# linnil1/KIR_graph

Hardware: AMD Instinct MI355X
Metric: typed 150 bp PE reads/s (pileup+EM) per GPU; achieved HBM GB/s vs roofline (higher is better)
Workload: dtype f64

## Files before the change

kir_graph_amd/csrc/gk_rowclass.hip:

```cpp
#include "gk_rowclass.h"

namespace {

constexpr int kThreads = 256;
constexpr int kGroup = 16, kDeep = 4;
constexpr int kRound = kGroup * kDeep;
constexpr int kCap = 256;
constexpr uint64_t kEmptyKey = ~0ull;
constexpr int kExpandCols = 8;

__device__ inline uint64_t mix64(uint64_t x) {
  x ^= x >> 30; x *= 0xBF58476D1CE4E5B9ull;
  x ^= x >> 27; x *= 0x94D049BB133111EBull;
  return x ^ (x >> 31);
}

template <class F>
__device__ inline uint32_t walk_round(const uint32_t* __restrict__ ids, const uint8_t* __restrict__ vflag, uint32_t k0,
                                      uint32_t mid, uint32_t e, int lane, int shift, uint32_t kept_before, F&& f) {
  uint32_t v[kDeep];
  uint8_t fl[kDeep];
  const uint32_t last = e - 1u;
#pragma unroll
  for (int j = 0; j < kDeep; ++j) {
    const uint32_t k = k0 + (uint32_t)lane + kGroup * j;
    v[j] = ids[k < e ? k : last];
  }
#pragma unroll
  for (int j = 0; j < kDeep; ++j) fl[j] = vflag[v[j]];
  uint32_t run = kept_before;
#pragma unroll
  for (int j = 0; j < kDeep; ++j) {
    const uint32_t k = k0 + (uint32_t)lane + kGroup * j;
    const bool positive = k < mid;
    const bool keep = k < e && !(fl[j] & (positive ? 1 : 2));
    const uint32_t mine = (uint32_t)(__ballot(keep) >> shift) & 0xFFFFu;
    if (keep) f((v[j] << 1) | (positive ? 0u : 1u), run + (uint32_t)__builtin_popcount(mine & ((1u << lane) - 1u)));
    run += (uint32_t)__builtin_popcount(mine);
  }
  return run;
}

__global__ __launch_bounds__(kThreads) void rowclass_keys(const int32_t* __restrict__ rows, int64_t n_rows,
                                                          const uint32_t* __restrict__ off,
                                                          const uint32_t* __restrict__ ids,
                                                          const uint8_t* __restrict__ vflag, uint64_t hash_mask,
                                                          unsigned long long* slot_key, uint32_t* slot_rep,
                                                          uint32_t slot_mask, uint32_t* __restrict__ slot_of) {
  const int lane = threadIdx.x & (kGroup - 1);
  const int shift = (threadIdx.x & 63) & ~(kGroup - 1);
  const int64_t i = ((int64_t)blockIdx.x * kThreads + threadIdx.x) / kGroup;
  const bool active = i < n_rows;
  uint32_t b = 0, mid = 0, e = 0;
  if (active) {
    const int64_t row = rows[i];
    b = off[4 * row]; mid = off[4 * row + 2]; e = off[4 * row + 4];
  }
  uint64_t h = 0;
  uint32_t n = 0;
  for (uint32_t k0 = b; k0 < e; k0 += kRound)
    n = walk_round(ids, vflag, k0, mid, e, lane, shift, n,
                   [&](uint32_t token, uint32_t rank) { h += mix64(((uint64_t)rank << 32) | token); });
  uint32_t lo = (uint32_t)h, hi = (uint32_t)(h >> 32);
#pragma unroll
  for (int d = kGroup / 2; d > 0; d >>= 1) {
    const uint64_t o = ((uint64_t)(uint32_t)__shfl_xor((int)hi, d, 64) << 32) | (uint32_t)__shfl_xor((int)lo, d, 64);
    h += o;
    lo = (uint32_t)h; hi = (uint32_t)(h >> 32);
  }
  if (!active || lane != 0) return;
  const unsigned long long key = mix64(h ^ n) & hash_mask & ~(1ull << 63);
  uint32_t s = (uint32_t)(key ^ (key >> 32)) & slot_mask;
  for (;;) {
    unsigned long long prev = __hip_atomic_load(&slot_key[s], __ATOMIC_RELAXED, __HIP_MEMORY_SCOPE_AGENT);
    if (prev == kEmptyKey) prev = atomicCAS(&slot_key[s], (unsigned long long)kEmptyKey, key);
    if (prev == kEmptyKey || prev == key) break;
    s = (s + 1u) & slot_mask;
  }
  if (__hip_atomic_load(&slot_rep[s], __ATOMIC_RELAXED, __HIP_MEMORY_SCOPE_AGENT) > (uint32_t)i)
    atomicMin(&slot_rep[s], (uint32_t)i);
  slot_of[i] = s;
}

__global__ __launch_bounds__(kThreads) void rowclass_verify(const int32_t* __restrict__ rows, int64_t n_rows,
                                                            const uint32_t* __restrict__ off,
                                                            const uint32_t* __restrict__ ids,
                                                            const uint8_t* __restrict__ vflag,
                                                            const uint32_t* __restrict__ slot_rep,
                                                            const uint32_t* __restrict__ slot_of,
                                                            uint32_t* __restrict__ is_rep, uint32_t* __restrict__ rep_of) {
  __shared__ uint32_t kept[kThreads / kGroup][kCap];
  const int lane = threadIdx.x & (kGroup - 1);
  const int shift = (threadIdx.x & 63) & ~(kGroup - 1);
  const int g = threadIdx.x / kGroup;
  const int64_t i = ((int64_t)blockIdx.x * kThreads + threadIdx.x) / kGroup;
  const bool active = i < n_rows;
  const uint32_t rep = active ? slot_rep[slot_of[i]] : 0u;
  const bool compare = active && rep < (uint32_t)i;
  uint32_t b = 0, mid = 0, e = 0, rb = 0, rmid = 0, re = 0;
  if (compare) {
    const int64_t row = rows[i], rrow = rows[rep];
    b = off[4 * row]; mid = off[4 * row + 2]; e = off[4 * row + 4];
    rb = off[4 * rrow]; rmid = off[4 * rrow + 2]; re = off[4 * rrow + 4];
  }
  uint32_t* const mine = kept[g];
  uint32_t n = 0, rn = 0;
  for (uint32_t k0 = b; k0 < e; k0 += kRound)
    n = walk_round(ids, vflag, k0, mid, e, lane, shift, n, [&](uint32_t token, uint32_t rank) {
      if (rank < (uint32_t)kCap) mine[rank] = token;
    });
  __builtin_amdgcn_fence(__ATOMIC_RELEASE, "wavefront");
  __builtin_amdgcn_wave_barrier();
  __builtin_amdgcn_fence(__ATOMIC_ACQUIRE, "wavefront");
  bool differs = false;
  for (uint32_t k0 = rb; k0 < re; k0 += kRound)
    rn = walk_round(ids, vflag, k0, rmid, re, lane, shift, rn, [&](uint32_t token, uint32_t rank) {
      if (rank < (uint32_t)kCap && mine[rank] != token) differs = true;
    });
  const bool any = ((__ballot(differs) >> shift) & 0xFFFFull) != 0ull;
  const bool same = compare && n == rn && n <= (uint32_t)kCap && !any;
  if (active && lane == 0) {
    is_rep[i] = same ? 0u : 1u;
    rep_of[i] = same ? rep : (uint32_t)i;
  }
}

__global__ __launch_bounds__(kThreads) void rowclass_rank(const int32_t* __restrict__ rep_idx,
                                                          const uint32_t* __restrict__ n_classes, int64_t n_rows,
                                                          const int32_t* __restrict__ rows, uint32_t* __restrict__ rank_of,
                                                          int32_t* __restrict__ rep_rows) {
  const int64_t c = (int64_t)blockIdx.x * kThreads + threadIdx.x;
  if (c >= n_rows || c >= (int64_t)*n_classes) return;
  const int32_t r = rep_idx[c];
  rank_of[r] = (uint32_t)c;
  rep_rows[c] = rows[r];
}

__global__ __launch_bounds__(kThreads) void rowclass_classof(const uint32_t* __restrict__ rep_of,
                                                             const uint32_t* __restrict__ rank_of, int64_t n_rows,
                                                             uint32_t* __restrict__ class_of) {
  const int64_t i = (int64_t)blockIdx.x * kThreads + threadIdx.x;
  if (i < n_rows) class_of[i] = rank_of[rep_of[i]];
}

__global__ __launch_bounds__(kThreads) void rowclass_expand(const double* __restrict__ Lc, int64_t ldc,
                                                            const uint32_t* __restrict__ class_of, int64_t n_rows,
                                                            int n_cols, double* __restrict__ L,
                                                            uint8_t* __restrict__ miss8, int64_t ldm) {
  const int a0 = (int)blockIdx.y * kExpandCols;
  const int n_a = min(kExpandCols, n_cols - a0);
  const int64_t r0 = 4 * ((int64_t)blockIdx.x * kThreads + threadIdx.x);
  if (r0 >= ldm) return;
  if (r0 >= n_rows) {
    for (int a = 0; a < n_a; ++a) *reinterpret_cast<uint32_t*>(miss8 + (int64_t)(a0 + a) * ldm + r0) = 0u;
    return;
  }
  const int n_r = (int)(n_rows - r0 < 4 ? n_rows - r0 : 4);
  uint32_t c[4];
  if (n_r == 4) {
    const uint4 q = *reinterpret_cast<const uint4*>(class_of + r0);
    c[0] = q.x; c[1] = q.y; c[2] = q.z; c[3] = q.w;
  } else {
#pragma unroll
    for (int j = 0; j < 4; ++j) c[j] = class_of[j < n_r ? r0 + j : n_rows - 1];
  }
  double v[4][kExpandCols];
#pragma unroll
  for (int j = 0; j < 4; ++j) {
    const double2* const src = reinterpret_cast<const double2*>(Lc + (int64_t)c[j] * ldc + a0);
#pragma unroll
    for (int q = 0; q < kExpandCols / 2; ++q) {
      const double2 x = src[q];
      v[j][2 * q] = x.x; v[j][2 * q + 1] = x.y;
    }
  }
#pragma unroll
  for (int a = 0; a < kExpandCols; ++a) {
    if (a >= n_a) break;
    uint32_t packed = 0;
#pragma unroll
    for (int j = 0; j < 4; ++j) {
      const double t = __builtin_fma(v[j][a], -1.0 / 3.0, 0.25);
      const uint32_t m = t < 100.0 ? (uint32_t)(int)t : 255u;
      if (j < n_r) packed |= m << (8 * j);
    }
    double* const dst = L + (int64_t)(a0 + a) * n_rows + r0;
    if (n_r == 4) {
#pragma unroll
      for (int j = 0; j < 4; ++j) dst[j] = v[j][a];
    } else {
#pragma unroll
      for (int j = 0; j < 4; ++j)
        if (j < n_r) dst[j] = v[j][a];
    }
    *reinterpret_cast<uint32_t*>(miss8 + (int64_t)(a0 + a) * ldm + r0) = packed;
  }
}

inline unsigned nblk(int64_t n) { return (unsigned)((n + kThreads - 1) / kThreads); }

}

int64_t gk_rowclass_ld(int n_cols) { return ((int64_t)n_cols + kExpandCols - 1) / kExpandCols * kExpandCols; }

int gk_rowclass_enqueue(gk_ctx* ctx, gk_tab* tab, const int32_t* d_rows, int64_t n_rows, const uint8_t* d_vflag,
                        gk_rowclass* rc) {
  GK_REQUIRE(ctx && tab && rc && d_rows && d_vflag && n_rows > 0 && n_rows <= 0x7FFFFFFFll, "bad row-class arguments");
  hipStream_t st = ctx->stream;
  const long bits = gk_test_hook_value("rowclass_hashbits", 63);
  const uint64_t hash_mask = bits >= 63 ? ~0ull : bits <= 0 ? 0ull : (1ull << bits) - 1ull;
  uint64_t n_slots = 64;
  while (n_slots < 2 * (uint64_t)n_rows) n_slots <<= 1;
  GkBlocks temps(ctx);
  char* slots = nullptr;
  uint32_t *slot_of = nullptr, *is_rep = nullptr, *rep_of = nullptr, *rank_of = nullptr, *class_of = nullptr, *n_classes = nullptr;
  int32_t *rep_idx = nullptr, *rep_rows = nullptr;
  const size_t per_row = (size_t)n_rows * sizeof(uint32_t);
  if (temps.take(&slots, (size_t)n_slots * 12) != hipSuccess || temps.take(&slot_of, per_row) != hipSuccess ||
      temps.take(&is_rep, per_row) != hipSuccess || temps.take(&rep_of, per_row) != hipSuccess ||
      temps.take(&rank_of, per_row) != hipSuccess || temps.take(&rep_idx, per_row) != hipSuccess ||
      temps.take(&rep_rows, per_row) != hipSuccess || temps.take(&class_of, per_row) != hipSuccess) {
    gk_set_error("out of device memory for the row classes");
    return GK_ERR_HIP;
  }
  unsigned long long* const slot_key = reinterpret_cast<unsigned long long*>(slots);
  uint32_t* const slot_rep = reinterpret_cast<uint32_t*>(slots + (size_t)n_slots * 8);
  if (hipMemsetAsync(slots, 0xFF, (size_t)n_slots * 12, st) != hipSuccess) {
    gk_set_error("row classes: clearing the slots failed");
    return GK_ERR_HIP;
  }
  const unsigned groups = nblk(n_rows * kGroup);
  GK_PROF(ctx, "rowclass_keys", GK_KERNEL(rowclass_keys, dim3(groups), dim3(kThreads), 0, st, d_rows, n_rows, tab->d_off,
                                          tab->d_ids, d_vflag, hash_mask, slot_key, slot_rep, (uint32_t)(n_slots - 1),
                                          slot_of));
  GK_PROF(ctx, "rowclass_verify", GK_KERNEL(rowclass_verify, dim3(groups), dim3(kThreads), 0, st, d_rows, n_rows,
                                            tab->d_off, tab->d_ids, d_vflag, slot_rep, slot_of, is_rep, rep_of));
  const int code = gk_compact_enqueue(ctx, is_rep, nullptr, n_rows, rep_idx, &n_classes, temps);
  if (code) return code;
  GK_PROF(ctx, "rowclass_rank", {
    GK_KERNEL(rowclass_rank, dim3(nblk(n_rows)), dim3(kThreads), 0, st, rep_idx, n_classes, n_rows, d_rows, rank_of,
              rep_rows);
    GK_KERNEL(rowclass_classof, dim3(nblk(n_rows)), dim3(kThreads), 0, st, rep_of, rank_of, n_rows, class_of);
  });
  if (hipGetLastError() != hipSuccess) {
    gk_set_error("row classes: a launch failed");
    return GK_ERR_HIP;
  }
  rc->rep_rows = rep_rows; rc->class_of = class_of; rc->n_classes = n_classes;
  rc->blocks = std::move(temps);
  return GK_OK;
}

int gk_rowclass_expand(gk_ctx* ctx, const gk_rowclass* rc, const double* Lc, int64_t ldc, int n_cols, int64_t n_rows,
                       double* L, uint8_t* miss8, int64_t ldm) {
  GK_REQUIRE(ctx && rc && rc->class_of && Lc && L && miss8 && n_cols > 0 && n_cols <= 65535 && n_rows > 0 &&
                 ldm >= n_rows && ldm % 64 == 0 && ldc == gk_rowclass_ld(n_cols), "bad expansion arguments");
  GK_PROF(ctx, "rowclass_expand", GK_KERNEL(rowclass_expand, dim3(nblk(ldm / 4), (unsigned)((n_cols + kExpandCols - 1) / kExpandCols)), dim3(kThreads), 0,
                                            ctx->stream, Lc, ldc, rc->class_of, n_rows, n_cols, L, miss8, ldm));
  GK_HIP(hipGetLastError());
  return GK_OK;
}

extern "C" int gk_row_classes(gk_ctx* ctx, gk_tab* tab, gk_dptr d_rows, int64_t n_rows, gk_dptr d_vflag, gk_dptr d_class_of,
                              int64_t* n_classes) {
  gk_bind(ctx);
  GK_REQUIRE(ctx && tab && n_classes && n_rows >= 0, "bad arguments");
  *n_classes = 0;
  if (n_rows == 0) return GK_OK;
  gk_rowclass rc;
  int code = gk_rowclass_enqueue(ctx, tab, gk_ptr<int32_t>(d_rows), n_rows, gk_ptr<uint8_t>(d_vflag), &rc);
  if (code) return code;
  if (d_class_of)
    (void)hipMemcpyAsync(gk_ptr<void>(d_class_of), rc.class_of, (size_t)n_rows * sizeof(uint32_t), hipMemcpyDeviceToDevice,
                         ctx->stream);
  uint32_t n = 0;
  GK_HIP(gk_fetch(ctx, &n, rc.n_classes, sizeof(uint32_t)));
  *n_classes = n;
  return GK_OK;
}
```

include/graphkir_hip.h:

```cpp
#ifndef GRAPHKIR_HIP_H
#define GRAPHKIR_HIP_H

#include <stddef.h>
#include <stdint.h>

#ifdef __cplusplus
extern "C" {
#endif

#define GK_ABI_VERSION 1

#define GK_OK 0
#define GK_ERR_NO_DEVICE (-1)
#define GK_ERR_HIP (-2)
#define GK_ERR_ARG (-3)
#define GK_ERR_ASSERT (-4)
#define GK_ERR_CAPACITY (-5)

#define GK_MAX_CIG 14
#define GK_MAX_MM 16
#define GK_MAX_INS 6
#define GK_MAX_EVENTS 22
#define GK_CIG_M 0
#define GK_CIG_I 1
// ... 97 lines not shown
                        gk_dptr d_gene_pos0, const gk_mate_wide* wide, const int64_t* spill_pair, int64_t n_spill,
                        gk_tab** out);
int gk_tab_from_csr(gk_ctx* ctx, int32_t n_var_total, int64_t n_valid, const uint32_t* off, const uint32_t* ids,
                    const uint8_t* pair_gene, const uint8_t* pair_nh, gk_tab** out);
int gk_tab_get_info(gk_tab* tab, gk_tab_info* info);
int gk_tab_destroy(gk_tab* tab);

int gk_select_gene(gk_ctx* ctx, gk_tab* tab, int gene, int multiple, gk_dptr d_rows_out, int64_t* n_out);
int gk_select_nonempty(gk_ctx* ctx, gk_tab* tab, gk_dptr d_rows, int64_t n_rows, gk_dptr d_vflag,
                       gk_dptr d_rows_out, int64_t* n_out);

int gk_variant_count(gk_ctx* ctx, gk_tab* tab, gk_dptr d_rows, int64_t n_rows, gk_dptr d_vflag,
                     gk_dptr d_cnt);
int gk_variant_count_range(gk_ctx* ctx, gk_tab* tab, gk_dptr d_rows, int64_t n_rows, gk_dptr d_vflag,
                           gk_dptr d_cnt, int32_t vbeg, int32_t vend);
int gk_variant_correct(gk_ctx* ctx, gk_tab* tab, gk_dptr d_cnt, gk_dptr d_vflag);
int gk_variant_surviving(gk_ctx* ctx, gk_tab* tab, gk_dptr d_cnt, gk_dptr d_vflag, int64_t max_out,
                         int32_t* ord_out, uint32_t* pos_out, uint32_t* neg_out, int64_t* n_out);

int gk_variant_surviving_gene(gk_ctx* ctx, gk_tab* tab, gk_dptr d_cnt, gk_dptr d_vflag, int32_t gene, int32_t vbeg,
                              int32_t vend, int64_t max_out, int32_t* ord_out, uint32_t* pos_out, uint32_t* neg_out,
                              int64_t* n_out);
int gk_sample_prepare(gk_ctx* ctx, gk_tab* tab, int32_t multiple, gk_dptr d_vflag, gk_dptr d_cnt, gk_dptr d_rows,
                      int64_t* gene_off_out);
int gk_sample_prepare_all(gk_ctx* ctx, gk_tab* tab, int32_t multiple, gk_dptr d_vflag, gk_dptr d_cnt, gk_dptr d_rows,
                          int64_t* gene_off_out, int64_t max_out, int32_t* ord_out, uint32_t* pos_out, uint32_t* neg_out,
                          int64_t* n_out, uint64_t* novel_key_out);
int gk_sample_prepare_exon(gk_ctx* ctx, gk_tab* tab, int32_t multiple, gk_dptr d_vflag, gk_dptr d_cnt, gk_dptr d_rows,
                           int64_t* gene_off_out, int64_t max_out, int32_t* ord_out, uint32_t* pos_out, uint32_t* neg_out,
                           int64_t* n_out);
int gk_sample_prepare_exon_from(gk_ctx* ctx, gk_tab* tab, int32_t multiple, gk_dptr d_vflag, gk_dptr d_cnt, gk_dptr d_rows,
                                int64_t* gene_off_out, int64_t max_out, int32_t* ord_out, uint32_t* pos_out,
                                uint32_t* neg_out, int64_t* n_out, gk_dptr d_cnt_full);

int gk_compat(gk_ctx* ctx, gk_tab* tab, gk_dptr d_rows, int64_t n_rows, gk_dptr d_vflag,
              int32_t vbeg, int32_t vend, gk_dptr d_mask, int32_t words, int32_t n_allele, int32_t keep_empty,
              gk_dptr d_probs, gk_dptr d_miss, gk_dptr d_nvar);

int gk_novel_assign(gk_ctx* ctx, gk_dptr d_probs, int64_t n_rows, int32_t n_cols, const uint32_t* col_entries,
                    int32_t n_entries, gk_dptr d_code, uint16_t* code_out, uint32_t* count_out, int32_t* first_out);
int gk_novel_confusion(gk_ctx* ctx, gk_tab* tab, gk_dptr d_rows, int64_t n_rows, gk_dptr d_code, gk_dptr d_vflag,
                       int32_t vbeg, int32_t vend, gk_dptr d_carry, const int32_t* entry_col, const int32_t* entry_slot,
                       int32_t n_entries, int32_t n_slots, uint64_t* totals_out, int64_t max_out, int32_t* slot_out,
                       int32_t* ord_out, uint32_t* count_out, uint64_t* key_out, int64_t* n_out);

int gk_lut_create(gk_ctx* ctx, int32_t log2_capacity, gk_lut** out);
int gk_lut_destroy(gk_lut* lut);
int gk_lut_collect(gk_lut* lut, gk_dptr d_vals, int64_t n);
int gk_lut_pending(gk_lut* lut, int32_t* n_total, int32_t* n_known);
int gk_lut_export(gk_lut* lut, int32_t first, int32_t count, double* keys_out);
int gk_lut_define(gk_lut* lut, int32_t first, int32_t count, const double* log_vals);
int gk_lut_apply(gk_lut* lut, gk_dptr d_in, gk_dptr d_out, int64_t n);
typedef int (*gk_log10_fn)(const double* values, int64_t n, double* out);
int gk_lut_resolve(gk_lut* lut, gk_log10_fn log10_fn, int32_t* n_new, int32_t* n_known, int32_t* n_undefined);
int gk_lut_resolve_stored(gk_lut* lut, gk_log10_fn log10_fn, int32_t* n_new, int32_t* n_known, int32_t* n_undefined);
int gk_lut_known(gk_lut* lut, int32_t* n_known);
int gk_compat_log(gk_ctx* ctx, gk_tab* tab, gk_dptr d_rows, int64_t n_rows, gk_dptr d_vflag,
                  int32_t vbeg, int32_t vend, gk_dptr d_mask, int32_t words, int32_t n_allele, int32_t keep_empty,
                  gk_lut* lut, gk_dptr d_log);

int gk_maxsum(gk_ctx* ctx, gk_dptr d_L, int64_t n_rows, int64_t ld, const int32_t* ids, int32_t n_sets,
              int32_t c_prev, const int32_t* cols, int32_t n_cols, double* out);
int gk_fraction(gk_ctx* ctx, gk_dptr d_L, int64_t n_rows, int64_t ld, const int32_t* ids,
                int32_t n_sets, int32_t c, double* frac_out);
int gk_setmax(gk_ctx* ctx, gk_dptr d_L, int64_t n_rows, int64_t ld, const int32_t* ids, int32_t n_sets,
              int32_t c, gk_dptr d_P);

int gk_compat_log_miss(gk_ctx* ctx, gk_tab* tab, gk_dptr d_rows, int64_t n_rows, gk_dptr d_vflag,
                       int32_t vbeg, int32_t vend, gk_dptr d_mask, int32_t words, int32_t n_allele,
                       int32_t keep_empty, gk_lut* lut, gk_dptr d_log, gk_dptr d_miss8, int64_t ldm, gk_dptr d_flags);
int gk_miss_colsum(gk_ctx* ctx, gk_dptr d_miss8, int64_t ldm, int32_t n_cols, gk_dptr d_msum);
int gk_compat_log_miss_cols(gk_ctx* ctx, gk_tab* tab, gk_dptr d_rows, int64_t n_rows, gk_dptr d_vflag,
                            int32_t vbeg, int32_t vend, gk_dptr d_mask, int32_t words, int32_t n_allele,
                            int32_t keep_empty, gk_lut* lut, const int32_t* table_cols, int32_t n_table_cols,
                            gk_dptr d_log, gk_dptr d_miss8, int64_t ldm, gk_dptr d_flags);
int gk_compat_log_miss_narrow(gk_ctx* ctx, gk_tab* tab, gk_dptr d_rows, int64_t n_rows, gk_dptr d_vflag,
                              int32_t vbeg, int32_t vend, gk_dptr d_mask, int32_t words, int32_t n_allele,
                              int32_t keep_empty, gk_lut* lut, const int32_t* table_cols, int32_t n_table_cols,
                              gk_dptr d_log, gk_dptr d_miss8, int64_t ldm, gk_dptr d_flags, gk_dptr d_msum);
int gk_compat_patch(gk_ctx* ctx, gk_lut* lut, gk_dptr d_log, int64_t n_rows, int32_t n_allele, gk_dptr d_miss8,
                    int64_t ldm, gk_dptr d_flags);
int gk_row_classes(gk_ctx* ctx, gk_tab* tab, gk_dptr d_rows, int64_t n_rows, gk_dptr d_vflag, gk_dptr d_class_of,
                   int64_t* n_classes);
int gk_compat_index(gk_ctx* ctx, gk_tab* tab, gk_dptr d_rows, int64_t n_rows, gk_dptr d_vflag, int32_t vbeg,
                    int32_t vend, gk_dptr d_mask, int32_t words, int32_t n_allele, int32_t keep_empty, gk_lut* lut,
                    gk_dptr d_lidx, gk_dptr d_miss8, int64_t ldm, gk_dptr d_flags);
int gk_expand_index(gk_ctx* ctx, gk_lut* lut, gk_dptr d_lidx, int64_t ldi, int64_t n_rows, int32_t n_allele, gk_dptr d_L,
                    int64_t ld);
int gk_bound_step(gk_ctx* ctx, gk_dptr d_miss8, int64_t ldm, int64_t n_rows, gk_dptr d_msum, const int32_t* ids,
                  int32_t n_sets, int32_t c_prev, const int32_t* cols, int32_t n_cols, const uint8_t* first,
                  int32_t top_n, int32_t cap, uint32_t* hdr_out, int32_t* idx_out, uint32_t* m_out);
int gk_bound_step_classes(gk_ctx* ctx, gk_dptr d_miss8, int64_t ldm, int64_t n_rows, gk_dptr d_class_of, int64_t n_classes,
                          gk_dptr d_msum, const int32_t* ids, int32_t n_sets, int32_t c_prev, const int32_t* cols,
                          int32_t n_cols, const uint8_t* first, int32_t top_n, int32_t cap, uint32_t* hdr_out,
                          int32_t* idx_out, uint32_t* m_out);
int gk_class_slice_plan(const uint32_t* plane_counts, int64_t want, int32_t* slices_out, int32_t capacity, int32_t* n_slices,
                        int64_t* plane_blk0_out);
int gk_setsum(gk_ctx* ctx, gk_dptr d_L, int64_t n_rows, int64_t ld, const int32_t* ids, int32_t n_sets, int32_t c,
              double* value_out, double* frac_out);
int gk_setsum_few(gk_ctx* ctx, gk_dptr d_L, int64_t n_rows, int64_t ld, const int32_t* ids, int32_t n_sets, int32_t c,
                  double* value_out, double* frac_out);
int gk_test_pool_fail(gk_ctx* ctx, int64_t nth, int64_t* live_out, int64_t* mallocs_out);

typedef int (*gk_argsort_fn)(const double* values, int64_t n, int64_t* order_out);
typedef struct gk_search gk_search;
int gk_search_run(gk_ctx* ctx, gk_dptr d_L, int64_t n_rows, int64_t ld, int32_t n_allele, gk_dptr d_miss8,
                  int64_t ldm, gk_dptr d_msum, const int32_t* cols, int32_t n_cols, int32_t n_steps, int32_t top_n,
                  gk_argsort_fn argsort, const double* colsum_in, gk_search** out);
typedef struct gk_gene_job {
  gk_dptr d_rows;
  int64_t n_rows;
  gk_dptr d_mask;
  gk_dptr d_L;
  gk_dptr d_miss8;
  int64_t ldm;
  gk_dptr d_msum;
  gk_dptr d_flags;
  gk_dptr d_lidx;
  int32_t vbeg, vend;
  int32_t words, n_allele;
  int32_t n_steps, top_n;
  int32_t bound_ok, passes;
  int32_t indexed, patches;
  int32_t table_of, n_step_cols;
  const int32_t* step_cols;
  const int32_t* step_cols_off;
  const int32_t* table_cols;
  int32_t n_table_cols;
} gk_gene_job;
int gk_sample_search(gk_ctx* ctx, gk_ctx** more_ctx, int32_t n_more, gk_tab* tab, gk_dptr d_vflag, gk_lut* lut,
                     gk_gene_job* jobs, int32_t n_jobs, gk_argsort_fn argsort, gk_log10_fn log10_fn, gk_search** out);
int gk_search_steps(gk_search* s, int32_t* n_steps);
int gk_search_info(gk_search* s, int32_t step, int32_t* n, int64_t* rows, int32_t* bounded);
int gk_search_copy(gk_search* s, int32_t step, double* value, double* sum_indv, int32_t* ids, double* frac);
int gk_search_export(gk_search* const* s, int32_t n, int64_t* totals, int64_t* meta, double* value, double* sum_indv,
                     double* frac, int32_t* ids);
int gk_search_colsum(gk_search* s, double* out);
int gk_search_log(gk_search* s, int64_t* out, int64_t capacity, int64_t* n_out);
int gk_search_destroy(gk_search* s);
int gk_site_verdict(const int64_t* pos, const int64_t* code, const uint8_t* negative, const int64_t* count, int64_t n,
                    int32_t cn, int32_t* homozygous);
int gk_site_verdict_tallies(const uint64_t* keys, int64_t n_keys, const int64_t* label_of_insert, int64_t n_insert,
                            const int32_t* ordinal, const uint32_t* positive, const uint32_t* negative, int64_t n,
                            int32_t cn, int32_t* homozygous);
int gk_site_verdict_genes(const uint64_t* keys, int64_t n_keys, const int64_t* label_of_insert, int64_t n_insert,
                          const int32_t* ordinal, const uint32_t* positive, const uint32_t* negative,
                          const int64_t* bounds, int32_t n_groups, const int32_t* cn, int32_t* homozygous);

int gk_em_sets(gk_ctx* ctx, gk_tab* tab, gk_dptr d_rows, int64_t n_rows, int32_t vbeg, int32_t vend,
               gk_dptr d_mask, int32_t words, gk_dptr d_sets_out );
int gk_em_distinct(gk_ctx* ctx, gk_dptr d_sets, int64_t n_rows, int32_t words, int32_t max_out,
                   uint32_t* sets_out, uint32_t* count_out, int32_t* n_out);
int gk_em_run(gk_ctx* ctx, const uint32_t* sets, const double* weight, int32_t n_sets, int32_t words,
              int32_t n_allele, int32_t iter_max, double diff_threshold, double* prob_out,
              int32_t* iters_out);
typedef struct gk_em_job {
  gk_dptr d_rows;
  int64_t n_rows;
  gk_dptr d_mask;
  int32_t vbeg, vend;
  int32_t words, n_allele;
  int32_t n_distinct, iterations;
} gk_em_job;
int gk_sample_em(gk_ctx* ctx, gk_tab* tab, gk_em_job* jobs, int32_t n_jobs, int32_t iter_max, double diff_threshold,
                 double* prob_out, int64_t* count_out);

// ... 112 lines not shown
```

kir_graph_amd/_lib.py:

```python
from __future__ import annotations

import ctypes as C
import threading
import os
from pathlib import Path

import numpy as np

LIB_NAME = "libgraphkir_hip.so"
_lib = None


class GkError(RuntimeError):
    """Error reported by the native library."""


class GkNoDevice(GkError):
    """No HIP device: the typing path cannot run (there is no CPU fallback)."""


_MM = np.dtype([("ref_off", "<u2"), ("base", "u1"), ("rsv", "u1")])
MATE_DTYPE = np.dtype([
    ("pos0", "<u4"), ("flag", "<u2"), ("ref", "u1"), ("nh", "u1"),
    ("nm", "u1"), ("n_cig", "u1"), ("n_mm", "u1"), ("n_ins", "u1"),
# ... 133 lines not shown
    "gk_bam_write_lines": (C.c_int, [C.c_char_p, C.c_char_p, C.c_int64, C.c_char_p, C.c_int64, C.c_void_p, C.c_int64,
                                     C.c_int32]),
    "gk_json_write_reads": (C.c_int, [C.c_char_p, C.c_char_p, C.c_int64, C.c_void_p, C.c_int64, C.c_void_p, C.c_int64,
                                      C.c_void_p, C.c_void_p, C.c_void_p, C.c_int64, C.c_void_p, C.c_int32,
                                      C.c_void_p, C.c_void_p]),
    "gk_bam_pack": (C.c_int, [C.c_void_p, C.c_void_p]),
    "gk_bam_next": (C.c_int, [C.c_void_p, C.c_void_p, C.c_int64, C.POINTER(C.c_int64)]),
    "gk_compat_log": (C.c_int, [C.c_void_p, C.c_void_p, C.c_uint64, C.c_int64, C.c_uint64, C.c_int32, C.c_int32,
                                C.c_uint64, C.c_int32, C.c_int32, C.c_int32, C.c_void_p, C.c_uint64]),
    "gk_maxsum": (C.c_int, [C.c_void_p, C.c_uint64, C.c_int64, C.c_int64, C.c_void_p, C.c_int32, C.c_int32,
                            C.c_void_p, C.c_int32, C.c_void_p]),
    "gk_fraction": (C.c_int, [C.c_void_p, C.c_uint64, C.c_int64, C.c_int64, C.c_void_p, C.c_int32, C.c_int32,
                              C.c_void_p]),
    "gk_setmax": (C.c_int, [C.c_void_p, C.c_uint64, C.c_int64, C.c_int64, C.c_void_p, C.c_int32, C.c_int32,
                            C.c_uint64]),
    "gk_packer_create": (C.c_int, [C.c_void_p, C.c_int32, C.c_void_p, C.c_int32, C.POINTER(C.c_void_p)]),
    "gk_packer_destroy": (C.c_int, [C.c_void_p]),
    "gk_packer_feed": (C.c_int, [C.c_void_p, C.c_char_p, C.c_size_t, C.c_int32]),
    "gk_packer_counts": (C.c_int, [C.c_void_p, C.POINTER(C.c_int64), C.POINTER(C.c_int64), C.POINTER(C.c_int64),
                                   C.POINTER(C.c_int64), C.POINTER(C.c_int64)]),
    "gk_packer_error": (C.c_int, [C.c_void_p, C.POINTER(C.c_int32), C.POINTER(C.c_int64)]),
    "gk_packer_records": (C.c_int, [C.c_void_p, C.c_void_p, C.c_void_p]),
    "gk_packer_set_output": (C.c_int, [C.c_void_p, C.c_void_p, C.c_int64]),
    "gk_packer_spilled": (C.c_int, [C.c_void_p, C.POINTER(C.c_int64)]),
    "gk_packer_spill_records": (C.c_int, [C.c_void_p, C.c_void_p, C.c_void_p]),
    "gk_packer_string": (C.c_char_p, [C.c_void_p, C.c_int64]),
    "gk_depth": (C.c_int, [C.c_void_p, C.c_void_p, C.c_uint64, C.c_int32, C.c_void_p, C.c_int32, C.c_void_p]),
    "gk_depth_compact": (C.c_int, [C.c_void_p, C.c_void_p, C.c_uint64, C.c_int32, C.c_void_p, C.c_int32, C.c_void_p]),
    "gk_depth_weighted": (C.c_int, [C.c_void_p, C.c_void_p, C.c_uint64, C.c_uint64, C.c_int32, C.c_void_p, C.c_int32, C.c_uint64,
                                    C.c_int64, C.c_int32, C.c_void_p, C.c_void_p, C.c_void_p, C.c_void_p, C.c_void_p]),
    "gk_depth_write_tsv": (C.c_int, [C.c_char_p, C.c_void_p, C.c_void_p, C.c_int32, C.c_void_p]),
    "gk_cn_fit": (C.c_int, [C.c_void_p, C.c_void_p, C.c_void_p, C.c_int32, C.c_void_p, C.c_int32, C.c_void_p,
                            C.c_int32, C.c_int32, C.c_double, C.c_void_p]),
    "gk_cn_assign": (C.c_int, [C.c_void_p, C.c_void_p, C.c_int32, C.c_double, C.c_void_p, C.c_int32, C.c_int32,
                               C.c_double, C.c_void_p]),
    "gk_em_sets": (C.c_int, [C.c_void_p, C.c_void_p, C.c_uint64, C.c_int64, C.c_int32, C.c_int32, C.c_uint64,
                             C.c_int32, C.c_uint64]),
    "gk_em_distinct": (C.c_int, [C.c_void_p, C.c_uint64, C.c_int64, C.c_int32, C.c_int32, C.c_void_p, C.c_void_p,
                                 C.POINTER(C.c_int32)]),
    "gk_compat_log_miss_cols": (C.c_int, [C.c_void_p, C.c_void_p, C.c_uint64, C.c_int64, C.c_uint64, C.c_int32, C.c_int32,
                                          C.c_uint64, C.c_int32, C.c_int32, C.c_int32, C.c_void_p, C.c_void_p, C.c_int32,
                                          C.c_uint64, C.c_uint64, C.c_int64, C.c_uint64]),
    "gk_compat_log_miss_narrow": (C.c_int, [C.c_void_p, C.c_void_p, C.c_uint64, C.c_int64, C.c_uint64, C.c_int32, C.c_int32,
                                            C.c_uint64, C.c_int32, C.c_int32, C.c_int32, C.c_void_p, C.c_void_p, C.c_int32,
                                            C.c_uint64, C.c_uint64, C.c_int64, C.c_uint64, C.c_uint64]),
    "gk_compat_log_miss": (C.c_int, [C.c_void_p, C.c_void_p, C.c_uint64, C.c_int64, C.c_uint64, C.c_int32, C.c_int32,
                                     C.c_uint64, C.c_int32, C.c_int32, C.c_int32, C.c_void_p, C.c_uint64, C.c_uint64,
                                     C.c_int64, C.c_uint64]),
    "gk_miss_colsum": (C.c_int, [C.c_void_p, C.c_uint64, C.c_int64, C.c_int32, C.c_uint64]),
    "gk_compat_index": (C.c_int, [C.c_void_p, C.c_void_p, C.c_uint64, C.c_int64, C.c_uint64, C.c_int32, C.c_int32,
                                  C.c_uint64, C.c_int32, C.c_int32, C.c_int32, C.c_void_p, C.c_uint64, C.c_uint64,
                                  C.c_int64, C.c_uint64]),
    "gk_expand_index": (C.c_int, [C.c_void_p, C.c_void_p, C.c_uint64, C.c_int64, C.c_int64, C.c_int32, C.c_uint64,
                                  C.c_int64]),
    "gk_bound_step": (C.c_int, [C.c_void_p, C.c_uint64, C.c_int64, C.c_int64, C.c_uint64, C.c_void_p, C.c_int32,
                                C.c_int32, C.c_void_p, C.c_int32, C.c_void_p, C.c_int32, C.c_int32, C.c_void_p,
                                C.c_void_p, C.c_void_p]),
    "gk_bound_step_classes": (C.c_int, [C.c_void_p, C.c_uint64, C.c_int64, C.c_int64, C.c_uint64, C.c_int64, C.c_uint64,
                                        C.c_void_p, C.c_int32, C.c_int32, C.c_void_p, C.c_int32, C.c_void_p, C.c_int32,
                                        C.c_int32, C.c_void_p, C.c_void_p, C.c_void_p]),
    "gk_class_slice_plan": (C.c_int, [C.c_void_p, C.c_int64, C.c_void_p, C.c_int32, C.c_void_p, C.c_void_p]),
    "gk_setsum": (C.c_int, [C.c_void_p, C.c_uint64, C.c_int64, C.c_int64, C.c_void_p, C.c_int32, C.c_int32,
                            C.c_void_p, C.c_void_p]),
    "gk_setsum_few": (C.c_int, [C.c_void_p, C.c_uint64, C.c_int64, C.c_int64, C.c_void_p, C.c_int32, C.c_int32,
                                C.c_void_p, C.c_void_p]),
    "gk_test_pool_fail": (C.c_int, [C.c_void_p, C.c_int64, C.POINTER(C.c_int64), C.POINTER(C.c_int64)]),
    "gk_search_run": (C.c_int, [C.c_void_p, C.c_uint64, C.c_int64, C.c_int64, C.c_int32, C.c_uint64, C.c_int64,
                                C.c_uint64, C.c_void_p, C.c_int32, C.c_int32, C.c_int32, C.c_void_p, C.c_void_p,
                                C.POINTER(C.c_void_p)]),
    "gk_sample_search": (C.c_int, [C.c_void_p, C.c_void_p, C.c_int32, C.c_void_p, C.c_uint64, C.c_void_p, C.c_void_p,
                                   C.c_int32, C.c_void_p, C.c_void_p, C.c_void_p]),
    "gk_lut_resolve": (C.c_int, [C.c_void_p, C.c_void_p, C.POINTER(C.c_int32), C.POINTER(C.c_int32),
                                 C.POINTER(C.c_int32)]),
    "gk_sample_prepare_exon": (C.c_int, [C.c_void_p, C.c_void_p, C.c_int32, C.c_uint64, C.c_uint64, C.c_uint64, C.c_void_p,
                                         C.c_int64, C.c_void_p, C.c_void_p, C.c_void_p, C.POINTER(C.c_int64)]),
    "gk_sample_prepare_exon_from": (C.c_int, [C.c_void_p, C.c_void_p, C.c_int32, C.c_uint64, C.c_uint64, C.c_uint64, C.c_void_p,
                                              C.c_int64, C.c_void_p, C.c_void_p, C.c_void_p, C.POINTER(C.c_int64), C.c_uint64]),
    "gk_sample_em": (C.c_int, [C.c_void_p, C.c_void_p, C.c_void_p, C.c_int32, C.c_int32, C.c_double, C.c_void_p, C.c_void_p]),
    "gk_mates_compact": (C.c_int, [C.c_void_p, C.c_uint64, C.c_int64, C.POINTER(C.c_uint64), C.POINTER(C.c_int64)]),
    "gk_mates_expand": (C.c_int, [C.c_void_p, C.c_uint64, C.c_int64, C.c_uint64]),
    "gk_mates_compact_size": (C.c_int, [C.c_void_p, C.c_int64, C.c_int32, C.POINTER(C.c_int64)]),
    "gk_mates_compact_host": (C.c_int, [C.c_void_p, C.c_int64, C.c_int32, C.c_void_p, C.c_int64]),
    "gk_row_classes": (C.c_int, [C.c_void_p, C.c_void_p, C.c_uint64, C.c_int64, C.c_uint64, C.c_uint64, C.POINTER(C.c_int64)]),
    "gk_compat_patch": (C.c_int, [C.c_void_p, C.c_void_p, C.c_uint64, C.c_int64, C.c_int32, C.c_uint64, C.c_int64, C.c_uint64]),
    "gk_lut_resolve_stored": (C.c_int, [C.c_void_p, C.c_void_p, C.POINTER(C.c_int32), C.POINTER(C.c_int32),
                                        C.POINTER(C.c_int32)]),
    "gk_lut_known": (C.c_int, [C.c_void_p, C.POINTER(C.c_int32)]),
    "gk_search_steps": (C.c_int, [C.c_void_p, C.POINTER(C.c_int32)]),
    "gk_search_info": (C.c_int, [C.c_void_p, C.c_int32, C.POINTER(C.c_int32), C.POINTER(C.c_int64),
                                 C.POINTER(C.c_int32)]),
    "gk_search_copy": (C.c_int, [C.c_void_p, C.c_int32, C.c_void_p, C.c_void_p, C.c_void_p, C.c_void_p]),
    "gk_search_export": (C.c_int, [C.c_void_p, C.c_int32, C.c_void_p, C.c_void_p, C.c_void_p, C.c_void_p, C.c_void_p, C.c_void_p]),
    "gk_search_colsum": (C.c_int, [C.c_void_p, C.c_void_p]),
    "gk_search_log": (C.c_int, [C.c_void_p, C.c_void_p, C.c_int64, C.POINTER(C.c_int64)]),
    "gk_search_destroy": (C.c_int, [C.c_void_p]),
    "gk_site_verdict_tallies": (C.c_int, [C.c_void_p, C.c_int64, C.c_void_p, C.c_int64, C.c_void_p, C.c_void_p, C.c_void_p,
                                         C.c_int64, C.c_int32, C.POINTER(C.c_int32)]),
    "gk_site_verdict_genes": (C.c_int, [C.c_void_p, C.c_int64, C.c_void_p, C.c_int64, C.c_void_p, C.c_void_p, C.c_void_p,
                                       C.c_void_p, C.c_int32, C.c_void_p, C.c_void_p]),
    "gk_site_verdict": (C.c_int, [C.c_void_p, C.c_void_p, C.c_void_p, C.c_void_p, C.c_int64, C.c_int32,
                                  C.POINTER(C.c_int32)]),
    "gk_comm_unique_id": (C.c_int, [C.c_void_p, C.c_size_t]),
    "gk_comm_create": (C.c_int, [C.c_void_p, C.c_void_p, C.c_size_t, C.c_int32, C.c_int32, C.POINTER(C.c_void_p)]),
    "gk_comm_destroy": (C.c_int, [C.c_void_p]),
    "gk_allgather_f64": (C.c_int, [C.c_void_p, C.c_void_p, C.c_void_p, C.c_int64]),
    "gk_allreduce_max_f64": (C.c_int, [C.c_void_p, C.c_void_p, C.c_int64]),
    "gk_comm_barrier": (C.c_int, [C.c_void_p]),
    "gk_host_alloc": (C.c_int, [C.c_size_t, C.POINTER(C.c_void_p)]),
    "gk_host_free": (C.c_int, [C.c_void_p]),
    "gk_h2d_async": (C.c_int, [C.c_void_p, C.c_uint64, C.c_void_p, C.c_size_t]),
    "gk_em_run": (C.c_int, [C.c_void_p, C.c_void_p, C.c_void_p, C.c_int32, C.c_int32, C.c_int32, C.c_int32,
                            C.c_double, C.c_void_p, C.POINTER(C.c_int32)]),
    "gk_em_bootstrap": (C.c_int, [C.c_void_p, C.c_void_p, C.c_int32, C.c_int32, C.c_uint64, C.c_int32, C.c_double,
                                  C.c_void_p, C.c_void_p, C.c_void_p]),
    "gk_boot_row_counts": (C.c_int, [C.c_void_p, C.c_int64, C.c_int32, C.c_int32, C.c_uint64, C.c_uint32, C.c_uint64,
                                     C.c_int64]),
    "gk_weighted_sums": (C.c_int, [C.c_void_p, C.c_uint64, C.c_int64, C.c_int64, C.c_int32, C.c_uint64, C.c_int64, C.c_int32,
                                   C.c_void_p]),
    "gk_call_fit": (C.c_int, [C.c_void_p, C.c_uint64, C.c_int64, C.c_int64, C.c_int32, C.c_void_p, C.c_int32, C.c_void_p,
                              C.c_void_p, C.c_void_p, C.c_uint64]),
    "gk_call_fit_extra": (C.c_int, [C.c_void_p, C.c_uint64, C.c_int64, C.c_int64, C.c_int32, C.c_uint64, C.c_void_p]),
    "gk_call_swap": (C.c_int, [C.c_void_p, C.c_uint64, C.c_int64, C.c_int64, C.c_int32, C.c_void_p, C.c_int32, C.c_void_p,
                               C.c_void_p, C.c_void_p, C.c_void_p, C.c_void_p, C.c_void_p, C.c_uint64]),
    "gk_call_coverage": (C.c_int, [C.c_void_p, C.c_void_p, C.c_uint64, C.c_uint64, C.c_uint64, C.c_int64, C.c_uint64, C.c_int64,
                                   C.c_int32, C.c_void_p, C.c_int32, C.c_int32, C.c_int64, C.c_void_p]),
}

EXPORTED = sorted(_SIGS)

ARGSORT_FN = C.CFUNCTYPE(C.c_int, C.POINTER(C.c_double), C.c_int64, C.POINTER(C.c_int64))


def _numpy_argsort(values, n, order_out):
    try:
        v = np.ctypeslib.as_array(values, shape=(n,))
        np.ctypeslib.as_array(order_out, shape=(n,))[:] = np.argsort(v)
        return 0
    except Exception:
        return 1


NUMPY_ARGSORT = ARGSORT_FN(_numpy_argsort)

LOG10_FN = C.CFUNCTYPE(C.c_int, C.POINTER(C.c_double), C.c_int64, C.POINTER(C.c_double))


def _numpy_log10(values, n, out):
    try:
        v = np.ctypeslib.as_array(values, shape=(n,))
        with np.errstate(divide="ignore"):
            np.ctypeslib.as_array(out, shape=(n,))[:] = np.log10(v)
        return 0
    except Exception:
        return 1


NUMPY_LOG10 = LOG10_FN(_numpy_log10)


def lib():
    global _lib
    if _lib is None:
        path = libPath()
        if not path.exists():
            raise GkError(
                f"{path} is missing: build it with `python -c 'import __graft_entry__ as g; g.build()'` "
# ... 221 lines not shown
```

Baseline: 617.6 million.

## Stage row-class expansion through a padded shared-memory tile for coalesced stores

The expand kernel now gathers a 128-row by 32-column tile of class likelihoods into padded LDS, with 16 lanes reading contiguous double2 pairs per row. After a barrier it writes L column-major with one row per lane, and writes miss8 as packed quads, so both output streams are fully coalesced. Before, each thread wrote 4 consecutive doubles per column with a large thread stride. The class-matrix leading dimension padding changes from 8 to 16 columns. This adds LDS use and a sync, and the gathered columns are clamped at ldc-2, so out-of-range columns reread valid data that is then masked.

Measured after the change: 583.9 million. -5.5%, worse.

```diff
diff --git a/kir_graph_amd/csrc/gk_rowclass.hip b/kir_graph_amd/csrc/gk_rowclass.hip
--- a/kir_graph_amd/csrc/gk_rowclass.hip
+++ b/kir_graph_amd/csrc/gk_rowclass.hip
@@ -7,7 +7,20 @@
 constexpr int kRound = kGroup * kDeep;
 constexpr int kCap = 256;
 constexpr uint64_t kEmptyKey = ~0ull;
-constexpr int kExpandCols = 8;
+constexpr int kTileRows = 128, kTileCols = 32;
+constexpr int kLdCols = 16;
+constexpr int kTileLd = kTileCols + 1;
+constexpr int kGatherLanes = kTileCols / 2;
+constexpr int kGatherRows = kThreads / kGatherLanes;
+constexpr int kGatherDeep = kTileRows / kGatherRows;
+constexpr int kOutGroups = kThreads / kTileRows;
+constexpr int kQuads = kTileRows / 4;
+constexpr int kMissGroups = kThreads / kQuads;
+static_assert(kTileCols % kLdCols == 0 && kThreads % kGatherLanes == 0 && kTileRows % kGatherRows == 0, "gather shape");
+static_assert(kThreads % kTileRows == 0 && kTileCols % kOutGroups == 0 && kTileRows % 64 == 0, "store shape of L");
+static_assert(kThreads % kQuads == 0 && kTileCols % kMissGroups == 0, "store shape of miss8");
+
+__device__ inline int64_t lower(int64_t a, int64_t b) { return a < b ? a : b; }
 
 __device__ inline uint64_t mix64(uint64_t x) {
   x ^= x >> 30; x *= 0xBF58476D1CE4E5B9ull;
@@ -147,53 +160,51 @@
                                                             const uint32_t* __restrict__ class_of, int64_t n_rows,
                                                             int n_cols, double* __restrict__ L,
                                                             uint8_t* __restrict__ miss8, int64_t ldm) {
-  const int a0 = (int)blockIdx.y * kExpandCols;
-  const int n_a = min(kExpandCols, n_cols - a0);
-  const int64_t r0 = 4 * ((int64_t)blockIdx.x * kThreads + threadIdx.x);
-  if (r0 >= ldm) return;
-  if (r0 >= n_rows) {
-    for (int a = 0; a < n_a; ++a) *reinterpret_cast<uint32_t*>(miss8 + (int64_t)(a0 + a) * ldm + r0) = 0u;
-    return;
-  }
-  const int n_r = (int)(n_rows - r0 < 4 ? n_rows - r0 : 4);
-  uint32_t c[4];
-  if (n_r == 4) {
-    const uint4 q = *reinterpret_cast<const uint4*>(class_of + r0);
-    c[0] = q.x; c[1] = q.y; c[2] = q.z; c[3] = q.w;
-  } else {
-#pragma unroll
-    for (int j = 0; j < 4; ++j) c[j] = class_of[j < n_r ? r0 + j : n_rows - 1];
-  }
-  double v[4][kExpandCols];
-#pragma unroll
-  for (int j = 0; j < 4; ++j) {
-    const double2* const src = reinterpret_cast<const double2*>(Lc + (int64_t)c[j] * ldc + a0);
-#pragma unroll
-    for (int q = 0; q < kExpandCols / 2; ++q) {
-      const double2 x = src[q];
-      v[j][2 * q] = x.x; v[j][2 * q + 1] = x.y;
+  __shared__ double tile[kTileRows][kTileLd];
+  const int t = (int)threadIdx.x;
+  const int a0 = (int)blockIdx.y * kTileCols;
+  const int64_t r0 = (int64_t)blockIdx.x * kTileRows;
+  {
+    const int cl = t % kGatherLanes, sub = t / kGatherLanes;
+    const int64_t col = lower((int64_t)a0 + 2 * cl, ldc - 2);
+    uint32_t c[kGatherDeep];
+    double2 x[kGatherDeep];
+#pragma unroll
+    for (int p = 0; p < kGatherDeep; ++p) c[p] = class_of[lower(r0 + sub + kGatherRows * p, n_rows - 1)];
+#pragma unroll
+    for (int p = 0; p < kGatherDeep; ++p) x[p] = *reinterpret_cast<const double2*>(Lc + (int64_t)c[p] * ldc + col);
+#pragma unroll
+    for (int p = 0; p < kGatherDeep; ++p) {
+      tile[sub + kGatherRows * p][2 * cl] = x[p].x;
+      tile[sub + kGatherRows * p][2 * cl + 1] = x[p].y;
     }
   }
-#pragma unroll
-  for (int a = 0; a < kExpandCols; ++a) {
-    if (a >= n_a) break;
-    uint32_t packed = 0;
-#pragma unroll
-    for (int j = 0; j < 4; ++j) {
-      const double t = __builtin_fma(v[j][a], -1.0 / 3.0, 0.25);
-      const uint32_t m = t < 100.0 ? (uint32_t)(int)t : 255u;
-      if (j < n_r) packed |= m << (8 * j);
+  __syncthreads();
+  {
+    const int r = t % kTileRows, ag = t / kTileRows;
+    const bool row_in = r0 + r < n_rows;
+#pragma unroll
+    for (int q = 0; q < kTileCols / kOutGroups; ++q) {
+      const int a = ag + kOutGroups * q;
+      const double v = tile[r][a];
+      if (row_in && a0 + a < n_cols) L[(int64_t)(a0 + a) * n_rows + r0 + r] = v;
     }
-    double* const dst = L + (int64_t)(a0 + a) * n_rows + r0;
-    if (n_r == 4) {
-#pragma unroll
-      for (int j = 0; j < 4; ++j) dst[j] = v[j][a];
-    } else {
-#pragma unroll
-      for (int j = 0; j < 4; ++j)
-        if (j < n_r) dst[j] = v[j][a];
+  }
+  {
+    const int rq = t % kQuads, ag = t / kQuads;
+    const int64_t rw = r0 + 4 * rq;
+#pragma unroll
+    for (int q = 0; q < kTileCols / kMissGroups; ++q) {
+      const int a = ag + kMissGroups * q;
+      uint32_t packed = 0;
+#pragma unroll
+      for (int j = 0; j < 4; ++j) {
+        const double u = __builtin_fma(tile[4 * rq + j][a], -1.0 / 3.0, 0.25);
+        const uint32_t m = u < 100.0 ? (uint32_t)(int)u : 255u;
+        packed |= (rw + j < n_rows ? m : 0u) << (8 * j);
+      }
+      if (rw < ldm && a0 + a < n_cols) *reinterpret_cast<uint32_t*>(miss8 + (int64_t)(a0 + a) * ldm + rw) = packed;
     }
-    *reinterpret_cast<uint32_t*>(miss8 + (int64_t)(a0 + a) * ldm + r0) = packed;
   }
 }
 
@@ -201,7 +212,7 @@
 
 }
 
-int64_t gk_rowclass_ld(int n_cols) { return ((int64_t)n_cols + kExpandCols - 1) / kExpandCols * kExpandCols; }
+int64_t gk_rowclass_ld(int n_cols) { return ((int64_t)n_cols + kLdCols - 1) / kLdCols * kLdCols; }
 
 int gk_rowclass_enqueue(gk_ctx* ctx, gk_tab* tab, const int32_t* d_rows, int64_t n_rows, const uint8_t* d_vflag,
                         gk_rowclass* rc) {
@@ -255,7 +266,7 @@
                        double* L, uint8_t* miss8, int64_t ldm) {
   GK_REQUIRE(ctx && rc && rc->class_of && Lc && L && miss8 && n_cols > 0 && n_cols <= 65535 && n_rows > 0 &&
                  ldm >= n_rows && ldm % 64 == 0 && ldc == gk_rowclass_ld(n_cols), "bad expansion arguments");
-  GK_PROF(ctx, "rowclass_expand", GK_KERNEL(rowclass_expand, dim3(nblk(ldm / 4), (unsigned)((n_cols + kExpandCols - 1) / kExpandCols)), dim3(kThreads), 0,
+  GK_PROF(ctx, "rowclass_expand", GK_KERNEL(rowclass_expand, dim3((unsigned)((ldm + kTileRows - 1) / kTileRows), (unsigned)((n_cols + kTileCols - 1) / kTileCols)), dim3(kThreads), 0,
                                             ctx->stream, Lc, ldc, rc->class_of, n_rows, n_cols, L, miss8, ldm));
   GK_HIP(hipGetLastError());
   return GK_OK;
```

## Stage row-class expansion through LDS tiles for coalesced column-major stores

Applied to the files above, without the earlier changes.

Rewrites the rowclass_expand kernel so each block gathers a 128-row by 32-column tile of class rows into shared memory, using wave shuffles to broadcast class ids and 16-byte loads, then writes the column-major L output with lane-contiguous rows. The old version had each thread write four scattered doubles per column. It also adds a padded slot swizzle to avoid LDS bank conflicts and an XCD-style block-index remap. A raw C entry point and a tile-query function are exported as well. The cost is extra shared-memory traffic and a barrier per block.

New measurement: 641.8 million before, 635.6 million after. About the same (-1.0%).

```diff
diff --git a/include/graphkir_hip.h b/include/graphkir_hip.h
--- a/include/graphkir_hip.h
+++ b/include/graphkir_hip.h
@@ -203,6 +203,9 @@
                     int64_t ldm, gk_dptr d_flags);
 int gk_row_classes(gk_ctx* ctx, gk_tab* tab, gk_dptr d_rows, int64_t n_rows, gk_dptr d_vflag, gk_dptr d_class_of,
                    int64_t* n_classes);
+int gk_rowclass_expand_raw(gk_ctx* ctx, gk_dptr d_Lc, int64_t ldc, gk_dptr d_class_of, int64_t n_rows, int32_t n_cols,
+                           gk_dptr d_L, gk_dptr d_miss8, int64_t ldm);
+void gk_rowclass_expand_tile(int32_t* rows, int32_t* cols);
 int gk_compat_index(gk_ctx* ctx, gk_tab* tab, gk_dptr d_rows, int64_t n_rows, gk_dptr d_vflag, int32_t vbeg,
                     int32_t vend, gk_dptr d_mask, int32_t words, int32_t n_allele, int32_t keep_empty, gk_lut* lut,
                     gk_dptr d_lidx, gk_dptr d_miss8, int64_t ldm, gk_dptr d_flags);
diff --git a/kir_graph_amd/_lib.py b/kir_graph_amd/_lib.py
--- a/kir_graph_amd/_lib.py
+++ b/kir_graph_amd/_lib.py
@@ -239,6 +239,9 @@
     "gk_mates_compact_size": (C.c_int, [C.c_void_p, C.c_int64, C.c_int32, C.POINTER(C.c_int64)]),
     "gk_mates_compact_host": (C.c_int, [C.c_void_p, C.c_int64, C.c_int32, C.c_void_p, C.c_int64]),
     "gk_row_classes": (C.c_int, [C.c_void_p, C.c_void_p, C.c_uint64, C.c_int64, C.c_uint64, C.c_uint64, C.POINTER(C.c_int64)]),
+    "gk_rowclass_expand_raw": (C.c_int, [C.c_void_p, C.c_uint64, C.c_int64, C.c_uint64, C.c_int64, C.c_int32, C.c_uint64,
+                                         C.c_uint64, C.c_int64]),
+    "gk_rowclass_expand_tile": (None, [C.POINTER(C.c_int32), C.POINTER(C.c_int32)]),
     "gk_compat_patch": (C.c_int, [C.c_void_p, C.c_void_p, C.c_uint64, C.c_int64, C.c_int32, C.c_uint64, C.c_int64, C.c_uint64]),
     "gk_lut_resolve_stored": (C.c_int, [C.c_void_p, C.c_void_p, C.POINTER(C.c_int32), C.POINTER(C.c_int32),
                                         C.POINTER(C.c_int32)]),
diff --git a/kir_graph_amd/csrc/gk_rowclass.hip b/kir_graph_amd/csrc/gk_rowclass.hip
--- a/kir_graph_amd/csrc/gk_rowclass.hip
+++ b/kir_graph_amd/csrc/gk_rowclass.hip
@@ -143,57 +143,83 @@
   if (i < n_rows) class_of[i] = rank_of[rep_of[i]];
 }
 
+constexpr int kTileRows = 128, kTileCols = 32;
+constexpr int kWaves = kThreads / 64;
+constexpr int kPieces = kTileCols / 2;
+constexpr int kRowsPerLoad = 64 / kPieces;
+constexpr int kWaveRows = kTileRows / kWaves;
+constexpr int kLoads = kWaveRows / kRowsPerLoad;
+constexpr int kSlotBytes = kTileCols * 8 + 16;
+constexpr int kWaveCols = 256 / kTileRows;
+constexpr int kPassCols = kWaveCols * kWaves;
+static_assert(kTileRows % 64 == 0 && 256 % kTileRows == 0 && kTileCols % kPassCols == 0 && kTileCols % kExpandCols == 0 &&
+                  kPieces <= 64 && 64 % kPieces == 0 && kWaveRows <= 64 && kWaveRows % kRowsPerLoad == 0,
+              "tile shape");
+
+__device__ inline int expand_slot(int r) { return (r & ~15) | ((r + (r >> 4)) & 15); }
+
 __global__ __launch_bounds__(kThreads) void rowclass_expand(const double* __restrict__ Lc, int64_t ldc,
                                                             const uint32_t* __restrict__ class_of, int64_t n_rows,
                                                             int n_cols, double* __restrict__ L,
                                                             uint8_t* __restrict__ miss8, int64_t ldm) {
-  const int a0 = (int)blockIdx.y * kExpandCols;
-  const int n_a = min(kExpandCols, n_cols - a0);
-  const int64_t r0 = 4 * ((int64_t)blockIdx.x * kThreads + threadIdx.x);
+  __shared__ __attribute__((aligned(16))) unsigned char tile[kTileRows * kSlotBytes];
+  const int lane = threadIdx.x & 63, wave = threadIdx.x >> 6;
+  const int a0 = (int)blockIdx.y * kTileCols;
+  const int a_end = min(kTileCols, n_cols - a0);
+  const int64_t row0 = ((int64_t)(blockIdx.x & 7u) * (gridDim.x >> 3) + (blockIdx.x >> 3)) * kTileRows;
+  if (row0 >= ldm) return;
+  const int g = lane >> 4;
+  const int rt = 64 * (g / kWaveCols) + 4 * (lane & 15);
+  const int64_t r0 = row0 + rt;
+  const int ac = wave * kWaveCols + g % kWaveCols;
+  if (row0 >= n_rows) {
+    if (r0 < ldm)
+      for (int al = ac; al < a_end; al += kPassCols)
+        *reinterpret_cast<uint32_t*>(miss8 + (int64_t)(a0 + al) * ldm + r0) = 0u;
+    return;
+  }
+  {
+    const int64_t rw = row0 + wave * kWaveRows + (lane < kWaveRows ? lane : kWaveRows - 1);
+    const uint32_t mine = class_of[rw < n_rows ? rw : n_rows - 1];
+    const int piece = lane % kPieces, sub = lane / kPieces;
+    const int64_t col = min((int64_t)a0 + 2 * piece, ldc - 2);
+    uint4 v[kLoads];
+#pragma unroll
+    for (int i = 0; i < kLoads; ++i) {
+      const uint32_t c = (uint32_t)__shfl((int)mine, i * kRowsPerLoad + sub, 64);
+      v[i] = *reinterpret_cast<const uint4*>(Lc + (int64_t)c * ldc + col);
+    }
+#pragma unroll
+    for (int i = 0; i < kLoads; ++i) {
+      const int r = wave * kWaveRows + i * kRowsPerLoad + sub;
+      *reinterpret_cast<uint4*>(tile + expand_slot(r) * kSlotBytes + piece * 16) = v[i];
+    }
+  }
+  __syncthreads();
+#pragma unroll
+  for (int h = 0; h < kTileRows / 64; ++h) {
+    const int r = 64 * h + lane;
+    if (row0 + r >= n_rows) break;
+    const unsigned char* const src = tile + expand_slot(r) * kSlotBytes;
+    double* const dst = L + (int64_t)a0 * n_rows + row0 + r;
+#pragma unroll 4
+    for (int al = wave; al < a_end; al += kWaves) dst[(int64_t)al * n_rows] = *reinterpret_cast<const double*>(src + al * 8);
+  }
   if (r0 >= ldm) return;
-  if (r0 >= n_rows) {
-    for (int a = 0; a < n_a; ++a) *reinterpret_cast<uint32_t*>(miss8 + (int64_t)(a0 + a) * ldm + r0) = 0u;
-    return;
-  }
   const int n_r = (int)(n_rows - r0 < 4 ? n_rows - r0 : 4);
-  uint32_t c[4];
-  if (n_r == 4) {
-    const uint4 q = *reinterpret_cast<const uint4*>(class_of + r0);
-    c[0] = q.x; c[1] = q.y; c[2] = q.z; c[3] = q.w;
-  } else {
-#pragma unroll
-    for (int j = 0; j < 4; ++j) c[j] = class_of[j < n_r ? r0 + j : n_rows - 1];
-  }
-  double v[4][kExpandCols];
-#pragma unroll
-  for (int j = 0; j < 4; ++j) {
-    const double2* const src = reinterpret_cast<const double2*>(Lc + (int64_t)c[j] * ldc + a0);
-#pragma unroll
-    for (int q = 0; q < kExpandCols / 2; ++q) {
-      const double2 x = src[q];
-      v[j][2 * q] = x.x; v[j][2 * q + 1] = x.y;
-    }
-  }
-#pragma unroll
-  for (int a = 0; a < kExpandCols; ++a) {
-    if (a >= n_a) break;
+  const unsigned char* src[4];
+#pragma unroll
+  for (int j = 0; j < 4; ++j) src[j] = tile + expand_slot(rt + j) * kSlotBytes;
+#pragma unroll 2
+  for (int al = ac; al < a_end; al += kPassCols) {
     uint32_t packed = 0;
 #pragma unroll
     for (int j = 0; j < 4; ++j) {
-      const double t = __builtin_fma(v[j][a], -1.0 / 3.0, 0.25);
+      const double t = __builtin_fma(*reinterpret_cast<const double*>(src[j] + al * 8), -1.0 / 3.0, 0.25);
       const uint32_t m = t < 100.0 ? (uint32_t)(int)t : 255u;
       if (j < n_r) packed |= m << (8 * j);
     }
-    double* const dst = L + (int64_t)(a0 + a) * n_rows + r0;
-    if (n_r == 4) {
-#pragma unroll
-      for (int j = 0; j < 4; ++j) dst[j] = v[j][a];
-    } else {
-#pragma unroll
-      for (int j = 0; j < 4; ++j)
-        if (j < n_r) dst[j] = v[j][a];
-    }
-    *reinterpret_cast<uint32_t*>(miss8 + (int64_t)(a0 + a) * ldm + r0) = packed;
+    *reinterpret_cast<uint32_t*>(miss8 + (int64_t)(a0 + al) * ldm + r0) = packed;
   }
 }
 
@@ -251,14 +277,39 @@
   return GK_OK;
 }
 
+namespace {
+
+int expand_launch(gk_ctx* ctx, const double* Lc, int64_t ldc, const uint32_t* class_of, int n_cols, int64_t n_rows,
+                  double* L, uint8_t* miss8, int64_t ldm) {
+  GK_REQUIRE(ctx && class_of && Lc && L && miss8 && n_cols > 0 && n_cols <= 65535 && n_rows > 0 &&
+                 n_rows <= 0x7FFFFFFFll && ldm >= n_rows && ldm % 64 == 0 && ldm / kTileRows < 0x7FFFFFFFll &&
+                 ldc == gk_rowclass_ld(n_cols), "bad expansion arguments");
+  const dim3 grid((unsigned)(((ldm + kTileRows - 1) / kTileRows + 7) / 8 * 8),
+                  (unsigned)((n_cols + kTileCols - 1) / kTileCols));
+  GK_PROF(ctx, "rowclass_expand", GK_KERNEL(rowclass_expand, grid, dim3(kThreads), 0, ctx->stream, Lc, ldc, class_of,
+                                            n_rows, n_cols, L, miss8, ldm));
+  GK_HIP(hipGetLastError());
+  return GK_OK;
+}
+
+}
+
 int gk_rowclass_expand(gk_ctx* ctx, const gk_rowclass* rc, const double* Lc, int64_t ldc, int n_cols, int64_t n_rows,
                        double* L, uint8_t* miss8, int64_t ldm) {
-  GK_REQUIRE(ctx && rc && rc->class_of && Lc && L && miss8 && n_cols > 0 && n_cols <= 65535 && n_rows > 0 &&
-                 ldm >= n_rows && ldm % 64 == 0 && ldc == gk_rowclass_ld(n_cols), "bad expansion arguments");
-  GK_PROF(ctx, "rowclass_expand", GK_KERNEL(rowclass_expand, dim3(nblk(ldm / 4), (unsigned)((n_cols + kExpandCols - 1) / kExpandCols)), dim3(kThreads), 0,
-                                            ctx->stream, Lc, ldc, rc->class_of, n_rows, n_cols, L, miss8, ldm));
-  GK_HIP(hipGetLastError());
-  return GK_OK;
+  GK_REQUIRE(rc, "bad expansion arguments");
+  return expand_launch(ctx, Lc, ldc, rc->class_of, n_cols, n_rows, L, miss8, ldm);
+}
+
+extern "C" int gk_rowclass_expand_raw(gk_ctx* ctx, gk_dptr d_Lc, int64_t ldc, gk_dptr d_class_of, int64_t n_rows,
+                                      int32_t n_cols, gk_dptr d_L, gk_dptr d_miss8, int64_t ldm) {
+  gk_bind(ctx);
+  return expand_launch(ctx, gk_ptr<double>(d_Lc), ldc, gk_ptr<uint32_t>(d_class_of), n_cols, n_rows, gk_ptr<double>(d_L),
+                       gk_ptr<uint8_t>(d_miss8), ldm);
+}
+
+extern "C" void gk_rowclass_expand_tile(int32_t* rows, int32_t* cols) {
+  if (rows) *rows = kTileRows;
+  if (cols) *cols = kTileCols;
 }
 
 extern "C" int gk_row_classes(gk_ctx* ctx, gk_tab* tab, gk_dptr d_rows, int64_t n_rows, gk_dptr d_vflag, gk_dptr d_class_of,
```
